# omerbt/TokenFlow

Measured on AMD Instinct MI355X. Metric: denoising-step hot-path frames/sec, higher is better.
Workload: dtype bf16

## Files before the change

### include/tokenflow_hip.h

```cpp
#ifndef TOKENFLOW_HIP_H
#define TOKENFLOW_HIP_H

#include <stddef.h>
#include <stdint.h>

#ifdef __cplusplus
extern "C" {
#endif

#define TF_ABI_VERSION 11

#define TF_API __attribute__((visibility("default")))

#define TF_BF16 0
#define TF_F16 1
#define TF_F32 2

#define TF_ATTN_INJECT 1
#define TF_ATTN_EXACT_SCALE 2
#define TF_ATTN_BANK_ONLY 4
#define TF_ATTN_SOURCE_ONLY 8
#define TF_ATTN_NO_SPLIT 16
#define TF_ATTN_FOLD_SCALE 64
#define TF_ATTN_OUT_F32 32
// ... 84 lines not shown
TF_API int tf_ext_attn_runs_merge_edits(void* out, int K, int Kq, int S, int H, int Dh, int n_runs, int n_edits,
                                 unsigned inject_mask, int64_t out_branch_stride, int64_t out_frame_stride,
                                 int flags, int dtype, void* ws, size_t ws_bytes, void* stream);

TF_API int tf_ext_attn_run_edits_plan(int K, int Kq, int run_n, int n_runs, int S, int H, int Dh, int n_edits,
                               unsigned inject_mask, int flags, int dtype, char* buf, size_t len);

TF_API int tf_head_pack(const void* const* slabs, const int64_t* frame_strides, int ns, void* send, int W, int Kl, int S,
                 int hd, int64_t ld, int elem_bytes, void* stream);

TF_API int tf_head_unpack(const void* recv, void* const* dsts, const int64_t* frame_strides, int nb, int W, int Kl, int S,
                   int hd, int64_t ld, int elem_bytes, void* stream);

TF_API int tf_window_halo_pack(const void* const* slabs, const int64_t* frame_strides, int ns, void* send, int n_seg,
                        const int* seg_f0, const int* seg_n, int Kl, int S, int D, int64_t ld, int dtype, void* stream);

TF_API int tf_frame_set_halo_pack(const void* const* slabs, const int64_t* frame_strides, int ns, void* send, int n_peer,
                           const uint64_t* masks, int Kl, int S, int D, int64_t ld, int dtype, void* stream);

TF_API int tf_edit_halo_pack(const void* const* slabs, const int64_t* frame_strides, int ns, void* send, int n_peer,
                      const uint64_t* masks, const void* const* q_slabs, const int64_t* q_frame_strides, int nq, void* q_stage,
                      int Kl, int S, int D, int64_t ld, int64_t ld_q, int dtype, void* stream);

TF_API int tf_pivot_inv_norm(const void* piv, float* inv_norm, int64_t rows, int D, int dtype,
                      void* stream);

TF_API size_t tf_nn_search_workspace_bytes(int64_t n_tgt, int S, int D, int P);

TF_API int tf_nn_search(const void* tgt, const void* piv, const float* inv_norm, int32_t* idx,
                 int64_t n_tgt, int S, int D, int P, int kf0, int kf1, int dtype,
                 void* ws, size_t ws_bytes, void* stream);

TF_API int tf_nn_search_plan(int64_t n_tgt, int S, int D, int P, int C, char* buf, size_t len);

TF_API int tf_gather_blend(const void* kf_out, const int32_t* idx, const float* w, const void* resid,
                    void* out, int K, int n, int S, int D, int P, int kf0, int kf1,
                    int in_dtype, int res_dtype, int out_dtype, void* stream);

TF_API size_t tf_nn_gather_blend_workspace_bytes(int64_t n_tgt, int S, int D, int P);

TF_API int tf_nn_gather_blend(const void* tgt, const void* piv, const float* inv_norm,
                       const void* kf_out, const float* w, const void* resid, void* out,
                       int K, int n, int S, int D, int P, int kf0, int kf1,
                       int search_dtype, int in_dtype, int res_dtype, int out_dtype,
                       void* ws, size_t ws_bytes, void* stream);

TF_API size_t tf_nn_gather_blend_chunks_workspace_bytes(int64_t n_tgt_chunk, int S, int D, int C);

TF_API int tf_nn_gather_blend_chunks(const void* tgt, const void* piv, const float* inv_norm, const void* kf_out,
                              const float* w, const void* resid, void* out, int K, int n, int C, int S, int D,
                              int slot0, int first_single, int search_dtype, int in_dtype, int res_dtype,
                              int out_dtype, int single_dtype, void* ws, size_t ws_bytes, void* stream);

TF_API int tf_nn_gather_blend_norm(const void* tgt, const void* piv, const float* inv_norm, const void* kf_out,
                            const float* w, const void* resid, void* out, int K, int n, int S, int D, int P, int kf0,
                            int kf1, int search_dtype, int in_dtype, int res_dtype, int out_dtype, const void* gamma,
                            const void* beta, float eps, int w_dtype, void* norm_out, int norm_dtype, void* ws,
                            size_t ws_bytes, void* stream);

TF_API int tf_nn_gather_blend_chunks_norm(const void* tgt, const void* piv, const float* inv_norm, const void* kf_out,
                                   const float* w, const void* resid, void* out, int K, int n, int C, int S, int D,
                                   int slot0, int first_single, int search_dtype, int in_dtype, int res_dtype,
                                   int out_dtype, int single_dtype, const void* gamma, const void* beta, float eps,
                                   int w_dtype, void* norm_out, int norm_dtype, void* ws, size_t ws_bytes,
                                   void* stream);

// ... 210 lines not shown
```

### tokenflow_amd/_lib.py

```python
import ctypes
import os

_HERE = os.path.dirname(os.path.abspath(__file__))
LIB_PATH = os.environ.get("TOKENFLOW_HIP_LIB") or os.path.join(_HERE, "libtokenflow_hip.so")

TF_BF16, TF_F16, TF_F32 = 0, 1, 2
TF_ATTN_INJECT, TF_ATTN_EXACT_SCALE, TF_ATTN_BANK_ONLY, TF_ATTN_SOURCE_ONLY, TF_ATTN_NO_SPLIT = 1, 2, 4, 8, 16
TF_ATTN_OUT_F32 = 32
TF_ATTN_FOLD_SCALE = 64
TF_ATTN_NO_FUSED, TF_ATTN_FUSED = 128, 1 << 17
TF_ATTN_HINT_QB2, TF_ATTN_PRECISE_P, TF_ATTN_NO_PRECISE_P = 1 << 14, 1 << 15, 1 << 16
TF_ATTN_MULTI_V, TF_ATTN_NO_MULTI_V = 1 << 19, 1 << 20
TF_ATTN_MULTI_V64 = 1 << 21
TF_ATTN_RUN_MULTI_V = 1 << 22
TF_ATTN_HINT_MIX = 1 << 18


def attn_hint(qw: int = 0, kw: int = 0, qb: int = 1) -> int:
    code = {0: 0, 1: 1, 2: 2, 4: 3, 8: 4}
    return (code[qw] << 8) | (code[kw] << 11) | (TF_ATTN_HINT_QB2 if qb == 2 else 0)


ABI_VERSION = 11
TF_MAX_EDITS = 8
TF_MAX_SEGMENTS = 8
TF_MAX_WINDOW_FRAMES = 64
TF_RANK_HEADS, TF_RANK_BANK, TF_RANK_SLOTS, TF_RANK_NO_HALO, TF_RANK_INV_NORM = 0, 1, 64, 16, 32
TF_RANK_BANK_RUNS = 2
TF_RANK_BANK_EDIT_RUNS = 3
TF_ERR_COMM = -6

_c = ctypes
_SIGNATURES = {
    "tf_abi_version": (_c.c_int, []),
    "tf_last_error": (_c.c_char_p, []),
    "tf_ext_attn_workspace_bytes": (_c.c_size_t, [_c.c_int] * 5),
    "tf_ext_attn_plan": (_c.c_int, [_c.c_int] * 7 + [_c.c_char_p, _c.c_size_t]),
    "tf_nn_search_plan": (_c.c_int, [_c.c_int64] + [_c.c_int] * 4 + [_c.c_char_p, _c.c_size_t]),
    "tf_ext_attn_fwd": (_c.c_int, [_c.c_void_p] * 4 + [_c.c_int] * 6 + [_c.c_int64, _c.c_float, _c.c_int, _c.c_int,
                                   _c.c_void_p, _c.c_size_t, _c.c_void_p]),
    "tf_ext_attn_fwd_strided": (_c.c_int, [_c.c_void_p] * 4 + [_c.c_int] * 6 + [_c.c_int64, _c.c_void_p, _c.c_float,
                                           _c.c_int, _c.c_int, _c.c_void_p, _c.c_size_t, _c.c_void_p]),
    "tf_ext_attn_edits_workspace_bytes": (_c.c_size_t, [_c.c_int] * 6),
    "tf_ext_attn_fwd_edits": (_c.c_int, [_c.c_void_p] * 4 + [_c.c_int] * 6 + [_c.c_int64, _c.c_void_p, _c.c_float,
                                         _c.c_int, _c.c_int, _c.c_int, _c.c_void_p, _c.c_size_t, _c.c_void_p]),
    "tf_ext_attn_edits_plan": (_c.c_int, [_c.c_int] * 8 + [_c.c_char_p, _c.c_size_t]),
    "tf_nn_gather_blend_chunks_edits": (_c.c_int, [_c.c_void_p] * 7 + [_c.c_int] * 13 + [_c.c_void_p, _c.c_size_t,
                                                   _c.c_void_p]),
    "tf_nn_gather_blend_chunks_norm_edits": (_c.c_int, [_c.c_void_p] * 7 + [_c.c_int] * 13 + [_c.c_void_p, _c.c_void_p,
                                                        _c.c_float, _c.c_int, _c.c_void_p, _c.c_int, _c.c_void_p,
                                                        _c.c_size_t, _c.c_void_p]),
    "tf_nn_gather_blend_edits_plan": (_c.c_int, [_c.c_int] * 6 + [_c.c_char_p, _c.c_size_t]),
    "tf_inject_copy_edits": (_c.c_int, [_c.c_void_p, _c.c_int64, _c.c_int, _c.c_int, _c.c_void_p]),
    "tf_ext_attn_fwd_edits_masked": (_c.c_int, [_c.c_void_p] * 4 + [_c.c_int] * 6 + [_c.c_int64, _c.c_void_p, _c.c_float,
                                                _c.c_int, _c.c_int, _c.c_int, _c.c_uint, _c.c_void_p, _c.c_size_t,
                                                _c.c_void_p]),
    "tf_ext_attn_edits_masked_plan": (_c.c_int, [_c.c_int] * 6 + [_c.c_uint, _c.c_int, _c.c_int, _c.c_char_p, _c.c_size_t]),
    "tf_ext_attn_fwd_edits_part": (_c.c_int, [_c.c_void_p] * 4 + [_c.c_int] * 6 + [_c.c_int64, _c.c_void_p, _c.c_float,
                                              _c.c_int, _c.c_int, _c.c_int, _c.c_uint, _c.c_int, _c.c_void_p, _c.c_size_t,
                                              _c.c_void_p]),
    "tf_ext_attn_edits_part_plan": (_c.c_int, [_c.c_int] * 6 + [_c.c_uint, _c.c_int, _c.c_int, _c.c_int, _c.c_char_p,
                                               _c.c_size_t]),
    "tf_inject_copy_edits_masked": (_c.c_int, [_c.c_void_p, _c.c_int64, _c.c_int, _c.c_uint, _c.c_int, _c.c_void_p]),
    "tf_ext_attn_runs_workspace_bytes": (_c.c_size_t, [_c.c_int] * 7),
    "tf_ext_attn_run": (_c.c_int, [_c.c_void_p] * 4 + [_c.c_int] * 10 + [_c.c_int64, _c.c_void_p, _c.c_float, _c.c_int,
                                   _c.c_int, _c.c_void_p, _c.c_size_t, _c.c_void_p]),
    "tf_ext_attn_runs_merge": (_c.c_int, [_c.c_void_p] + [_c.c_int] * 6 + [_c.c_int64, _c.c_int64, _c.c_int, _c.c_int,
                                          _c.c_void_p, _c.c_size_t, _c.c_void_p]),
    "tf_ext_attn_run_plan": (_c.c_int, [_c.c_int] * 9 + [_c.c_char_p, _c.c_size_t]),
    "tf_ext_attn_runs_edits_workspace_bytes": (_c.c_size_t, [_c.c_int] * 8),
    "tf_ext_attn_run_edits": (_c.c_int, [_c.c_void_p] * 4 + [_c.c_int] * 10 + [_c.c_int64, _c.c_void_p, _c.c_float, _c.c_int,
# ... 155 lines not shown
```

### tokenflow_amd/csrc/nn_search.hip

```cpp
#include <stdlib.h>

#include <type_traits>

#include "tf_common.h"

namespace {

template <int BK>
__device__ __forceinline__ int swz_off(int row, int piece) {
    if constexpr (BK == 64) return row * 128 + ((piece ^ ((row >> 1) & 7)) << 4);
    return row * (BK * 2) + ((piece ^ (row & 15)) << 4);
}

template <typename T>
__global__ __launch_bounds__(256) void pivot_inv_norm_kernel(const typename T::elem* __restrict__ piv,
                                                             float* __restrict__ inv_norm, int64_t rows, int D) {
    const int lane = threadIdx.x & 63;
    const int64_t wave = (int64_t)blockIdx.x * 4 + (threadIdx.x >> 6);
    const int64_t nwaves = (int64_t)gridDim.x * 4;
    for (int64_t r = wave; r < rows; r += nwaves) {
        const float inv = tf_row_inv_norm<T>(piv + r * D, D, lane);
        if (lane == 0) inv_norm[r] = inv;
    }
}

template <typename T, int WN, int BK, int TM>
__global__ __launch_bounds__(256) void nn_search_kernel(const typename T::elem* __restrict__ tgt,
                                                        const typename T::elem* __restrict__ piv,
                                                        const float* __restrict__ inv_norm,
                                                        int32_t* __restrict__ idx_out,
                                                        NnPartial* __restrict__ part_out, int64_t n_tgt, int S,
                                                        int D, int kf0, int kf1, int tiles_per_split, NnChunks ch) {
    typedef typename T::vec8 vec8;
    constexpr int TN = 64 * WN;
// ... 669 lines not shown
#pragma unroll
            for (int tt = 0; tt < TT; ++tt) {
                const float sc = acc[tt][r] * w;
                if (sc > best_v[tt]) {
                    best_v[tt] = sc;
                    best_i[tt] = (mt0 + mt) * TMR + rl;
                }
            }
        }
        if (has_next) stage_write(mt + 1);
        asm volatile("s_waitcnt vmcnt(0)" ::: "memory");
        __syncthreads();
    }
#pragma unroll
    for (int tt = 0; tt < TT; ++tt) {
        const float ov = __shfl_xor(best_v[tt], 32);
        const int oi = __shfl_xor(best_i[tt], 32);
        float bv = best_v[tt];
        int bi = best_i[tt];
        if (ov > bv || (ov == bv && oi < bi)) {
            bv = ov;
            bi = oi;
        }
        bi = bi < S ? bi : S - 1;
        if (hi == 0 && t_row[tt] < t_end) {
            if (part_out)
                part_out[((int64_t)blockIdx.z * gridDim.y + p) * n_tgt + t_row[tt]] = NnPartial{bv, bi};
            else
                idx_out[(int64_t)p * n_tgt + t_row[tt]] = bi;
        }
    }
}

template <typename T, int DK, int TJ = 4>
__global__ __launch_bounds__(256, TJ == 4 ? 2 : 3) void nn_search_rbs_kernel(const typename T::elem* __restrict__ tgt,
                                                               const typename T::elem* __restrict__ piv,
                                                               const float* __restrict__ inv_norm,
                                                               int32_t* __restrict__ idx_out,
                                                               NnPartial* __restrict__ part_out, int64_t n_tgt, int S,
                                                               int kf0, int kf1, int tiles_per_split, NnChunks ch) {
    typedef typename T::elem E;
    typedef typename T::vec8 vec8;
    constexpr int D = 16 * DK;
    constexpr int KS32 = D / 32;
    static_assert(D % 32 == 0 && (D / 8) % 8 == 0, "32-wide k-steps; the swizzle permutes inside groups of 8 pieces");
    constexpr int TMR = 32;
    constexpr int NPIECE = TMR * D * 2 / 1024;
    static_assert(NPIECE % 4 == 0, "pieces split evenly over the 4 waves");
    constexpr int A_ELEMS = TMR * D;

    extern __shared__ __attribute__((aligned(16))) unsigned char smem[];
    float* sInv = reinterpret_cast<float*>(smem + 2 * A_ELEMS * sizeof(E));

    const int tid = threadIdx.x;
    const int lane = tid & 63;
    const int wave = tid >> 6;
    const int g = lane >> 4;
    const int n16 = lane & 15;
    const int p = blockIdx.y;
    const int chunk = blockIdx.x / ch.ppc;
    if (p == 1 && nn_chunk_single(ch, chunk)) return;
    const int kf = (p == 0 ? kf0 : kf1) + chunk;
    const E* pv = piv + (int64_t)kf * S * D;
    const float* inv = inv_norm + (int64_t)kf * S;
    const int64_t t_end = (chunk + 1) * (int64_t)ch.nS;
    int64_t t_row[TJ];
#pragma unroll
    for (int j = 0; j < TJ; ++j)
        t_row[j] = chunk * (int64_t)ch.nS + (int64_t)(blockIdx.x - chunk * ch.ppc) * (64 * TJ) + wave * (16 * TJ) + 16 * j + n16;

    const int n_mt_all = (S + TMR - 1) / TMR;
    const int mt0 = blockIdx.z * tiles_per_split;
    const int n_mt = min(tiles_per_split, n_mt_all - mt0);

    vec8 fb[TJ][KS32];
#pragma unroll
    for (int j = 0; j < TJ; ++j) {
        const E* tp = tgt + (t_row[j] < t_end ? t_row[j] : t_end - 1) * D + 8 * g;
#pragma unroll
        for (int t = 0; t < KS32; ++t) fb[j][t] = __builtin_bit_cast(vec8, ld16(tp + 32 * t));
    }

    typedef __attribute__((address_space(3))) void* lds_ptr;
    typedef const __attribute__((address_space(1))) void* glb_ptr;
    const int wave_u = __builtin_amdgcn_readfirstlane(wave);
    int a_off[NPIECE / 4];
#pragma unroll
    for (int i = 0; i < NPIECE / 4; ++i) {
        const int o = (wave_u + 4 * i) * 1024 + lane * 16;
        const int r = o / (2 * D), pos = (o - r * 2 * D) >> 4;
        a_off[i] = r * D + ((pos ^ ((r >> 1) & 7)) << 3);
    }
    float rinv = 0.f;
    const unsigned lds0 = (unsigned)(size_t)(lds_ptr)smem;
    auto stage_load = [&](int mt) {
        const E* tile = pv + (int64_t)(mt0 + mt) * TMR * D;
#pragma unroll
        for (int i = 0; i < NPIECE / 4; ++i) {
            const unsigned dst = __builtin_amdgcn_readfirstlane(lds0 + (mt & 1) * (A_ELEMS * (int)sizeof(E)) + (wave_u + 4 * i) * 1024);
            unsigned keep;
            asm volatile("s_mov_b32 %0, m0\n\ts_mov_b32 m0, %2\n\ts_nop 0\n\tglobal_load_lds_dwordx4 %1, off\n\ts_mov_b32 m0, %0"
                         : "=&s"(keep)
                         : "v"((glb_ptr)(tile + a_off[i])), "s"(dst)
                         : "memory");
        }
        if (tid < TMR) {
            int row = (mt0 + mt) * TMR + tid;
            rinv = inv[row < S ? row : S - 1];
        }
    };
    auto stage_write = [&](int mt) {
        if (tid < TMR) sInv[(mt & 1) * TMR + tid] = rinv;
    };
    auto tile_done = [&]() {
        asm volatile("" : "+v"(rinv));
        asm volatile("s_waitcnt vmcnt(0)" ::: "memory");
        __syncthreads();
    };

    constexpr int ROW_BYTES = D * (int)sizeof(E);
    constexpr int HALF_BYTES = 16 * ROW_BYTES;
    constexpr int A_BYTES = A_ELEMS * (int)sizeof(E);
    constexpr int RING = TJ == 4 ? 3 : 5;
    static_assert(TMR == 32 && sizeof(E) == 2, "two 16-row halves whose rows 16 i + n16 share (r >> 1) & 7; 8 elements per 16-B piece");
    static_assert(KS32 % 2 == 0, "k-steps pair up into groups of 8 pieces");
    static_assert((KS32 / 2 - 1) * 128 + HALF_BYTES + A_BYTES < 65536, "every fragment offset fits ds_read's 16-bit immediate");
    static_assert(RING - 1 <= KS32, "the ring's prologue stays inside phase A");
    const int fa_base[2] = {n16 * ROW_BYTES + ((g ^ ((n16 >> 1) & 7)) << 4), n16 * ROW_BYTES + (((4 + g) ^ ((n16 >> 1) & 7)) << 4)};
    auto frag = [&](const int (&cur)[2], int k) {
        const int t = k % KS32, i = k / KS32;
        return __builtin_bit_cast(vec8, ld16(smem + cur[t & 1] + (t >> 1) * 128 + i * HALF_BYTES));
    };

    float best_v[TJ];
    int best_i[TJ];
#pragma unroll
    for (int j = 0; j < TJ; ++j) best_v[j] = -INFINITY, best_i[j] = 0;
    stage_load(0);
    stage_write(0);
#pragma unroll
    for (int j = 0; j < TJ; ++j)
#pragma unroll
        for (int t = 0; t < KS32; ++t) asm volatile("" : "+v"(fb[j][t]));
    asm volatile("" ::"s"(idx_out), "s"(part_out));
    tile_done();
    constexpr int EPG = TJ / 2;
    static_assert(TJ % 2 == 0 && EPG * (KS32 - 2) >= 4 * TJ, "a half-tile's fold fits beside the inner groups of a phase");
    auto fold1 = [&](const f32x4 (&a)[TJ], const f32x4 w, const int row0, int e) {
        const int r = e / TJ, j = e % TJ;
        asm volatile("" : "+v"(best_v[j]), "+v"(best_i[j]));
        const float sc = a[j][r] * w[r];
        if (sc > best_v[j]) {
            best_v[j] = sc;
            best_i[j] = row0 + r;
        }
        asm volatile("" : "+v"(best_v[j]), "+v"(best_i[j]));
    };
    f32x4 acc0[TJ], acc1[TJ];
#pragma unroll
    for (int j = 0; j < TJ; ++j) acc1[j] = f32x4{-INFINITY, -INFINITY, -INFINITY, -INFINITY};
    f32x4 w0, w1 = f32x4{1.f, 1.f, 1.f, 1.f};
    int row0, row1 = 0;
    vec8 fa[RING];
    int cur[2];
    auto group = [&](int k, f32x4 (&acc)[TJ], const f32x4 (&accf)[TJ], const f32x4 wf, const int rowf) {
        const int t = k % KS32;
        const bool read = k + RING - 1 < 2 * KS32;
        if (read) fa[(k + RING - 1) % RING] = frag(cur, k + RING - 1);
#pragma unroll
        for (int j = 0; j < TJ; ++j)
            acc[j] = T::mfma16(fa[k % RING], fb[j][t], t == 0 ? f32x4{0.f, 0.f, 0.f, 0.f} : acc[j]);
        if (t >= 1 && t <= (4 * TJ) / EPG) {
#pragma unroll
            for (int e = (t - 1) * EPG; e < t * EPG; ++e) fold1(accf, wf, rowf, e);
        }
        if (read) __builtin_amdgcn_sched_group_barrier(0x100, 1, 0);
#pragma unroll
        for (int j = 0; j < TJ; ++j) {
            __builtin_amdgcn_sched_group_barrier(0x008, 1, 0);
            __builtin_amdgcn_sched_group_barrier(0x002, 2, 0);
        }
        __builtin_amdgcn_sched_barrier(0);
    };
    for (int mt = 0; mt < n_mt; ++mt) {
        const bool has_next = mt + 1 < n_mt;
        const int buf = (mt & 1) * A_BYTES;
        cur[0] = fa_base[0] + buf, cur[1] = fa_base[1] + buf;
        const float* si = sInv + (mt & 1) * TMR + 4 * g;
#pragma unroll
        for (int k = 0; k < RING - 1; ++k) fa[k] = frag(cur, k);
        w0 = *reinterpret_cast<const f32x4*>(si);
        if (has_next) stage_load(mt + 1);
        row0 = (mt0 + mt) * TMR + 4 * g;
        __builtin_amdgcn_sched_barrier(0);
#pragma unroll
        for (int k = 0; k < KS32; ++k) group(k, acc0, acc1, w1, row1);
        w1 = *reinterpret_cast<const f32x4*>(si + 16);
#pragma unroll
        for (int k = KS32; k < 2 * KS32; ++k) group(k, acc1, acc0, w0, row0);
        row1 = row0 + 16;
        if (has_next) stage_write(mt + 1);
        tile_done();
    }
#pragma unroll
    for (int e = 0; e < 4 * TJ; ++e) fold1(acc1, w1, row1, e);
#pragma unroll
    for (int j = 0; j < TJ; ++j) {
        float bv = best_v[j];
        int bi = best_i[j];
#pragma unroll
        for (int o_ = 16; o_ <= 32; o_ <<= 1) {
            const float ov = __shfl_xor(bv, o_);
            const int oi = __shfl_xor(bi, o_);
            if (ov > bv || (ov == bv && oi < bi)) {
                bv = ov;
                bi = oi;
            }
        }
        bi = bi < S ? bi : S - 1;
        if (g == 0 && t_row[j] < t_end) {
            if (part_out)
                part_out[((int64_t)blockIdx.z * gridDim.y + p) * n_tgt + t_row[j]] = NnPartial{bv, bi};
            else
                idx_out[(int64_t)p * n_tgt + t_row[j]] = bi;
        }
    }
}

__global__ __launch_bounds__(256) void nn_finalize_kernel(const NnPartial* __restrict__ part,
                                                          int32_t* __restrict__ idx_out, int64_t total, int splits) {
    const int64_t g = (int64_t)blockIdx.x * 256 + threadIdx.x;
    if (g >= total) return;
    NnPartial b = part[g];
    for (int s = 1; s < splits; ++s) {
        const NnPartial c = part[(int64_t)s * total + g];
        if (c.v > b.v || (c.v == b.v && c.i < b.i)) b = c;
    }
    idx_out[g] = b.i;
}

enum NnKernel {
    NN_RB,
    NN_RB2,
    NN_WIDE,
    NN_BK64,
    NN_BK128,
    NN_DEEP,
    NN_GLDS
};
struct NnPlan {
    int kern;
    int64_t panels;
    int splits, tiles_per_split;
};

static int nn_min_wgs(int C) {
    static const int env = [] {
// ... 86 lines not shown
    auto kern = nn_search_kernel<T, WN, BK, TM>;
    (void)hipFuncSetAttribute(reinterpret_cast<const void*>(kern), hipFuncAttributeMaxDynamicSharedMemorySize, (int)lds);
    const NnChunks ch = nn_chunks(n_tgt, (int)pl.panels, single_mask);
    hipLaunchKernelGGL(kern, grid, dim3(256), lds, st, reinterpret_cast<const typename T::elem*>(tgt),
                       reinterpret_cast<const typename T::elem*>(piv), inv_norm, idx,
                       (splits > 1 || !fin) ? ws : nullptr, n_tgt * C, S, D, kf0, kf1, tps, ch);
    TF_LAUNCH_CHECK("tf_nn_search");
    return (fin && splits > 1) ? finalize(ws, idx, n_tgt * C * P, splits, st) : 0;
}

template <typename T>
int launch_nn_glds(const void* tgt, const void* piv, const float* inv_norm, int32_t* idx, NnPartial* ws, int64_t n_tgt,
                   int S, int D, int P, int kf0, int kf1, hipStream_t st, bool fin, int C, uint64_t single_mask) {
    constexpr size_t lds = 2 * (256 + 256) * 64 * 2 + 2 * 256 * 4 + 4 * 256 * 8;
    static_assert(lds <= 160 * 1024, "LDS");
    const NnPlan pl = nn_plan(n_tgt, S, D, P, C);
    const int splits = pl.splits, tps = pl.tiles_per_split;
    dim3 grid((unsigned)(pl.panels * C), (unsigned)P, (unsigned)splits);
    if (tf_plan_note("glds[splits=%d%s]", splits, C > 1 ? ",chunks" : "")) return (fin && splits > 1) ? finalize(ws, idx, n_tgt * C * P, splits, st) : 0;
#ifndef TF_TUNE_NN_NO_GLDS_SH
    auto kern = nn_search_glds_kernel<T, true>;
#else
    auto kern = nn_search_glds_kernel<T, false>;
#endif
    (void)hipFuncSetAttribute(reinterpret_cast<const void*>(kern), hipFuncAttributeMaxDynamicSharedMemorySize, (int)lds);
    const NnChunks ch = nn_chunks(n_tgt, (int)pl.panels, single_mask);
    hipLaunchKernelGGL(kern, grid, dim3(512), lds, st, reinterpret_cast<const typename T::elem*>(tgt),
                       reinterpret_cast<const typename T::elem*>(piv), inv_norm, idx,
                       (splits > 1 || !fin) ? ws : nullptr, n_tgt * C, S, D, kf0, kf1, tps, ch);
    TF_LAUNCH_CHECK("tf_nn_search");
    return (fin && splits > 1) ? finalize(ws, idx, n_tgt * C * P, splits, st) : 0;
}

template <typename T, int DK>
int launch_nn_rb(const void* tgt, const void* piv, const float* inv_norm, int32_t* idx, NnPartial* ws, int64_t n_tgt,
                 int S, int P, int kf0, int kf1, hipStream_t st, bool fin, int C, uint64_t single_mask) {
    constexpr int D = 16 * DK;
    const size_t lds = 2 * 32 * (D + 8) * 2 + 2 * 32 * 4;
    const NnPlan pl = nn_plan(n_tgt, S, D, P, C);
    const int splits = pl.splits, tps = pl.tiles_per_split;
    dim3 grid((unsigned)(pl.panels * C), (unsigned)P, (unsigned)splits);
    const NnChunks ch = nn_chunks(n_tgt, (int)pl.panels, single_mask);
    if (pl.kern == NN_RB2) {
        const size_t lds_g = 2 * 32 * D * 2 + 2 * 32 * 4;
#ifndef TF_TUNE_NN_NO_RBS
        if (tf_plan_note("rbs<TJ=4>[splits=%d%s]", splits, C > 1 ? ",chunks" : "")) return (fin && splits > 1) ? finalize(ws, idx, n_tgt * C * P, splits, st) : 0;
        hipLaunchKernelGGL((nn_search_rbs_kernel<T, DK>), grid, dim3(256), lds_g, st,
                           reinterpret_cast<const typename T::elem*>(tgt), reinterpret_cast<const typename T::elem*>(piv),
                           inv_norm, idx, (splits > 1 || !fin) ? ws : nullptr, n_tgt * C, S, kf0, kf1, tps, ch);
        TF_LAUNCH_CHECK("tf_nn_search");
        return (fin && splits > 1) ? finalize(ws, idx, n_tgt * C * P, splits, st) : 0;
#endif
        if (tf_plan_note("rbg<TT=2>[splits=%d%s]", splits, C > 1 ? ",chunks" : "")) return (fin && splits > 1) ? finalize(ws, idx, n_tgt * C * P, splits, st) : 0;
        hipLaunchKernelGGL((nn_search_rbg_kernel<T, DK, 2>), grid, dim3(256), lds_g, st,
                           reinterpret_cast<const typename T::elem*>(tgt), reinterpret_cast<const typename T::elem*>(piv),
                           inv_norm, idx, (splits > 1 || !fin) ? ws : nullptr, n_tgt * C, S, kf0, kf1, tps, ch);
        TF_LAUNCH_CHECK("tf_nn_search");
        return (fin && splits > 1) ? finalize(ws, idx, n_tgt * C * P, splits, st) : 0;
    }
    static const bool dma = [] { const char* e = getenv("TF_NN_RB_GLDS"); return !e || atoi(e) != 0; }();
    if (dma && S % 32 == 0) {
        const size_t lds_g = 2 * 32 * D * 2 + 2 * 32 * 4;
#ifndef TF_TUNE_NN_NO_RBS
        if (tf_plan_note("rbs<TJ=2>[splits=%d%s]", splits, C > 1 ? ",chunks" : "")) return (fin && splits > 1) ? finalize(ws, idx, n_tgt * C * P, splits, st) : 0;
        hipLaunchKernelGGL((nn_search_rbs_kernel<T, DK, 2>), grid, dim3(256), lds_g, st,
                           reinterpret_cast<const typename T::elem*>(tgt), reinterpret_cast<const typename T::elem*>(piv),
                           inv_norm, idx, (splits > 1 || !fin) ? ws : nullptr, n_tgt * C, S, kf0, kf1, tps, ch);
        TF_LAUNCH_CHECK("tf_nn_search");
        return (fin && splits > 1) ? finalize(ws, idx, n_tgt * C * P, splits, st) : 0;
#endif
        if (tf_plan_note("rbg<TT=1>[splits=%d%s]", splits, C > 1 ? ",chunks" : "")) return (fin && splits > 1) ? finalize(ws, idx, n_tgt * C * P, splits, st) : 0;
        hipLaunchKernelGGL((nn_search_rbg_kernel<T, DK>), grid, dim3(256), lds_g, st,
                           reinterpret_cast<const typename T::elem*>(tgt), reinterpret_cast<const typename T::elem*>(piv),
                           inv_norm, idx, (splits > 1 || !fin) ? ws : nullptr, n_tgt * C, S, kf0, kf1, tps, ch);
        TF_LAUNCH_CHECK("tf_nn_search");
        return (fin && splits > 1) ? finalize(ws, idx, n_tgt * C * P, splits, st) : 0;
    }
    if (tf_plan_note("rb[splits=%d%s]", splits, C > 1 ? ",chunks" : "")) return (fin && splits > 1) ? finalize(ws, idx, n_tgt * C * P, splits, st) : 0;
    hipLaunchKernelGGL((nn_search_rb_kernel<T, DK>), grid, dim3(256), lds, st,
                       reinterpret_cast<const typename T::elem*>(tgt), reinterpret_cast<const typename T::elem*>(piv),
                       inv_norm, idx, (splits > 1 || !fin) ? ws : nullptr, n_tgt * C, S, kf0, kf1, tps, ch);
    TF_LAUNCH_CHECK("tf_nn_search");
    return (fin && splits > 1) ? finalize(ws, idx, n_tgt * C * P, splits, st) : 0;
}

template <typename T>
int dispatch_nn(const void* tgt, const void* piv, const float* inv_norm, int32_t* idx, NnPartial* ws, int64_t n_tgt,
                int S, int D, int P, int kf0, int kf1, hipStream_t st, bool fin, int C = 1, uint64_t single_mask = 0) {
    TF_ARG(n_tgt <= (int64_t)INT32_MAX, TF_ERR_SHAPE, "tf_nn_search: %lld targets per chunk (< 2^31)", (long long)n_tgt);
    switch (nn_plan(n_tgt, S, D, P, C).kern) {
        case NN_RB:
        case NN_RB2:
            return launch_nn_rb<T, 20>(tgt, piv, inv_norm, idx, ws, n_tgt, S, P, kf0, kf1, st, fin, C, single_mask);
        case NN_GLDS:
            return launch_nn_glds<T>(tgt, piv, inv_norm, idx, ws, n_tgt, S, D, P, kf0, kf1, st, fin, C, single_mask);
        case NN_WIDE:
            return launch_nn<T, 2, 64, 128>(tgt, piv, inv_norm, idx, ws, n_tgt, S, D, P, kf0, kf1, st, fin, C, single_mask);
        case NN_DEEP:
            return launch_nn<T, 1, 256, 64>(tgt, piv, inv_norm, idx, ws, n_tgt, S, D, P, kf0, kf1, st, fin, C, single_mask);
        case NN_BK128:
// ... 6 lines not shown
}

extern "C" int tf_pivot_inv_norm(const void* piv, float* inv_norm, int64_t rows, int D, int dtype, void* stream) {
    TF_ARG(piv && inv_norm, TF_ERR_NULL, "tf_pivot_inv_norm: null pointer");
    TF_ARG(dtype == TF_BF16 || dtype == TF_F16, TF_ERR_DTYPE, "tf_pivot_inv_norm: dtype %d (bf16/f16 only)", dtype);
    TF_ARG(rows > 0 && D > 0 && D % 8 == 0, TF_ERR_SHAPE, "tf_pivot_inv_norm: rows=%lld D=%d (D %% 8 == 0)",
           (long long)rows, D);
    TF_ARG(tf_aligned16(piv), TF_ERR_ALIGN, "tf_pivot_inv_norm: piv not 16-byte aligned");
    hipStream_t st = reinterpret_cast<hipStream_t>(stream);
    const unsigned grid = (unsigned)((rows + 3) / 4 < 4096 ? (rows + 3) / 4 : 4096);
    if (dtype == TF_BF16)
        hipLaunchKernelGGL(pivot_inv_norm_kernel<BF16>, dim3(grid), dim3(256), 0, st,
                           reinterpret_cast<const __bf16*>(piv), inv_norm, rows, D);
    else
        hipLaunchKernelGGL(pivot_inv_norm_kernel<F16>, dim3(grid), dim3(256), 0, st,
                           reinterpret_cast<const _Float16*>(piv), inv_norm, rows, D);
    TF_LAUNCH_CHECK("tf_pivot_inv_norm");
    return 0;
}

extern "C" int tf_nn_search_plan(int64_t n_tgt, int S, int D, int P, int C, char* buf, size_t len) {
    TF_ARG(n_tgt > 0 && S > 0 && D > 0 && D % 8 == 0 && (P == 1 || P == 2) && C >= 1 && (C == 1 || P == 2), TF_ERR_SHAPE,
           "tf_nn_search_plan: n_tgt=%lld S=%d D=%d P=%d C=%d", (long long)n_tgt, S, D, P, C);
    TfPlanRec rec{buf, len, 0, 0};
    if (buf && len) buf[0] = 0;
    tf_plan_rec = &rec;
    const int rc = dispatch_nn<BF16>(nullptr, nullptr, nullptr, nullptr, nullptr, n_tgt, S, D, P, 0, 1, nullptr, C == 1, C, 0);
    tf_plan_rec = nullptr;
    if (rc) return rc;
    TF_ARG(rec.used < len, TF_ERR_WORKSPACE, "tf_nn_search_plan: the plan needs %zu bytes", rec.used + 1);
    return rec.n;
}

extern "C" size_t tf_nn_search_workspace_bytes(int64_t n_tgt, int S, int D, int P) {
    if (n_tgt <= 0 || S <= 0 || D <= 0 || P <= 0) return 0;
    const NnPlan pl = nn_plan(n_tgt, S, D, P);
    const size_t bytes = pl.splits > 1 ? (size_t)pl.splits * P * n_tgt * sizeof(NnPartial) : 0;
    return bytes < 256 ? 256 : bytes;
}

extern "C" int tf_nn_search(const void* tgt, const void* piv, const float* inv_norm, int32_t* idx, int64_t n_tgt,
                            int S, int D, int P, int kf0, int kf1, int dtype, void* ws, size_t ws_bytes,
                            void* stream) {
    TF_ARG(tgt && piv && inv_norm && idx && ws, TF_ERR_NULL, "tf_nn_search: null pointer");
    TF_ARG(dtype == TF_BF16 || dtype == TF_F16, TF_ERR_DTYPE, "tf_nn_search: dtype %d (bf16/f16 only)", dtype);
    TF_ARG(n_tgt > 0 && S > 0 && D > 0 && D % 8 == 0 && (P == 1 || P == 2) && kf0 >= 0 && (P == 1 || kf1 >= 0),
           TF_ERR_SHAPE, "tf_nn_search: n_tgt=%lld S=%d D=%d P=%d kf=(%d,%d)", (long long)n_tgt, S, D, P, kf0, kf1);
    TF_ARG(tf_aligned16(tgt) && tf_aligned16(piv) && tf_aligned16(ws) && tf_aligned16(inv_norm), TF_ERR_ALIGN,
           "tf_nn_search: inputs not 16-byte aligned (inv_norm included: the LDS-DMA kernel fetches it in 16-byte pieces)");
    TF_ARG(ws_bytes >= tf_nn_search_workspace_bytes(n_tgt, S, D, P), TF_ERR_WORKSPACE,
           "tf_nn_search: workspace %zu < %zu bytes", ws_bytes, tf_nn_search_workspace_bytes(n_tgt, S, D, P));
    hipStream_t st = reinterpret_cast<hipStream_t>(stream);
    NnPartial* part = reinterpret_cast<NnPartial*>(ws);
    return dtype == TF_BF16 ? dispatch_nn<BF16>(tgt, piv, inv_norm, idx, part, n_tgt, S, D, P, kf0, kf1, st, true)
                            : dispatch_nn<F16>(tgt, piv, inv_norm, idx, part, n_tgt, S, D, P, kf0, kf1, st, true);
}

int tf_nn_search_partials(const void* tgt, const void* piv, const float* inv_norm, NnPartial* part, int64_t n_tgt,
                          int S, int D, int P, int kf0, int kf1, int dtype, hipStream_t st, int* splits, int C,
                          uint64_t single_mask) {
    *splits = nn_plan(n_tgt, S, D, P, C).splits;
    return dtype == TF_BF16
               ? dispatch_nn<BF16>(tgt, piv, inv_norm, nullptr, part, n_tgt, S, D, P, kf0, kf1, st, false, C, single_mask)
               : dispatch_nn<F16>(tgt, piv, inv_norm, nullptr, part, n_tgt, S, D, P, kf0, kf1, st, false, C, single_mask);
}

// ... 4 lines not shown
```

### tokenflow_amd/ops.py

```python
import ctypes
import os
from typing import Optional, Sequence

import torch

from . import _lib

_DT = {torch.bfloat16: _lib.TF_BF16, torch.float16: _lib.TF_F16, torch.float32: _lib.TF_F32}


def _need_gpu(*ts):
    dev = None
    for t in ts:
        if t is None:
            continue
        if not t.is_cuda:
            raise _lib.TokenflowHipError(
                "tokenflow_amd ops run on MI355X only: got a CPU tensor (there is no CPU fallback)")
        if dev is None:
            dev = t.device
        elif t.device != dev:
            raise _lib.TokenflowHipError(f"tokenflow_amd ops: tensors on different devices ({dev} and {t.device})")
    return dev

# ... 256 lines not shown
    if part not in ("bank", "all"):
        raise ValueError(f"attn_frame_sets_part_plan: part {part!r} (\"bank\" or \"all\": the source part is set-free)")
    tab = _frame_sets("attn_frame_sets_part_plan", sets, K, Kq, int(q_frame0))
    flags = _attn_flags(inject, part, out_dtype == torch.float32, False, no_split, fused, hints)
    return _plan_tokens("tf_ext_attn_frame_sets_part_plan", _lib.load().tf_ext_attn_frame_sets_part_plan, K, Kq, int(q_frame0), S,
                        heads, dh, flags, _DT[dtype], ctypes.cast(tab, ctypes.c_void_p))


def attn_frame_sets_edits_plan(K: int, sets, S: int, heads: int, dh: int, n_edits: int, inject_mask: int,
                               dtype: torch.dtype = torch.bfloat16, out_dtype: Optional[torch.dtype] = None,
                               no_split: Optional[bool] = None, fused: Optional[bool] = None, multi_v: Optional[bool] = None,
                               multi_v64: Optional[bool] = None, hints: int = 0) -> list:
    tab = _frame_sets("attn_frame_sets_edits_plan", sets, K, K)
    mask = _edit_mask("attn_frame_sets_edits_plan", inject_mask, n_edits)
    flags = _attn_flags(False, "all", out_dtype == torch.float32, False, no_split, fused, hints) | _multi_v_bits(multi_v, multi_v64)
    return _plan_tokens("tf_ext_attn_frame_sets_edits_plan", _lib.load().tf_ext_attn_frame_sets_edits_plan, K, K, 0, S, heads,
                        dh, int(n_edits), mask, flags, _DT[dtype], ctypes.cast(tab, ctypes.c_void_p))


def _single_mask(what: str, mask, C: int) -> int:
    m = int(mask)
    if not 1 <= C <= 64 or m < 0 or m >> C:
        raise ValueError(f"{what}: single_mask {m:#x} over {C} chunks (1 .. 64 chunks, no bit at or above them)")
    return m


def propagate_segments_plan(n: int, n_chunks: int, S: int, D: int, single_mask: int) -> list:
    return _plan_tokens("tf_nn_gather_blend_segments_plan", _lib.load().tf_nn_gather_blend_segments_plan, int(n),
                        int(n_chunks), S, D, _single_mask("propagate_segments_plan", single_mask, int(n_chunks)))


def nn_plan(n_tgt: int, S: int, D: int, P: int, C: int = 1) -> list:
    return _plan_tokens("tf_nn_search_plan", _lib.load().tf_nn_search_plan, int(n_tgt), S, D, P, C)


def ext_attn(q: torch.Tensor, k: torch.Tensor, v: torch.Tensor, heads: int, scale: float,
             inject: bool, out: Optional[torch.Tensor] = None, q_frame0: int = 0,
             fold_scale: Optional[bool] = None, part: str = "all",
             out_dtype: Optional[torch.dtype] = None, no_split: Optional[bool] = None,
             fused: Optional[bool] = None, hints: int = 0) -> torch.Tensor:
    dev = _need_gpu(q, k, v, out)
    lib = _lib.load()
    B, S, D = k.shape
    Bq = q.shape[0]
    if B % 3 or Bq % 3 or D % heads or q.shape[1:] != k.shape[1:] or v.shape != k.shape:
        raise ValueError(f"ext_attn: bad shapes q{tuple(q.shape)} k{tuple(k.shape)} v{tuple(v.shape)} heads {heads}")
    K, Kq, dh = B // 3, Bq // 3, D // heads
    dt = _DT.get(q.dtype)
    if dt is None or dt == _lib.TF_F32 or k.dtype != q.dtype or v.dtype != q.dtype:
        raise TypeError(f"ext_attn: q/k/v must share dtype bf16 or f16, got {q.dtype},{k.dtype},{v.dtype}")

    def rows(t):
        if t.stride(-1) != 1 or t.stride(0) != S * t.stride(1):
            t = t.contiguous()
        return t
    q, k, v = rows(q), rows(k), rows(v)
    ld = q.stride(1)
    if k.stride(1) != ld or v.stride(1) != ld:
        q, k, v = q.contiguous(), k.contiguous(), v.contiguous()
        ld = D
    if out_dtype is None:
        out_dtype = out.dtype if out is not None else q.dtype
    if out_dtype not in (q.dtype, torch.float32):
        raise TypeError(f"ext_attn: out_dtype {out_dtype} (the input dtype or float32)")
    if out is None:
        out = torch.empty(Bq, S, D, dtype=out_dtype, device=q.device)
# ... 1214 lines not shown
```

Measured before the change: 1654.

## Balance nearest-neighbour search work across resident workgroups with flattened tile runs

Adds a balanced mode for the row-block nearest-neighbour search kernel. The (chunk, pivot, panel, tile) space is flattened into equal-length runs sized to the number of resident workgroups, so each workgroup walks consecutive tiles across pivot-frame and panel boundaries. At each boundary it emits a partial result and reloads target rows only when they change. Block indices are remapped across the eight XCDs. The aim is to cut tail imbalance and partially filled waves when the split grid does not match CU occupancy, at the cost of more complex control flow, duplicated partial writes for split slots, and a device-attribute query.

```diff
diff --git a/include/tokenflow_hip.h b/include/tokenflow_hip.h
--- a/include/tokenflow_hip.h
+++ b/include/tokenflow_hip.h
@@ -140,6 +140,8 @@
                  void* ws, size_t ws_bytes, void* stream);
 
 TF_API int tf_nn_search_plan(int64_t n_tgt, int S, int D, int P, int C, char* buf, size_t len);
+
+TF_API int tf_nn_search_partition(int64_t n_tgt, int S, int D, int P, int C, uint64_t single_mask, int cus, int* out);
 
 TF_API int tf_gather_blend(const void* kf_out, const int32_t* idx, const float* w, const void* resid,
                     void* out, int K, int n, int S, int D, int P, int kf0, int kf1,
diff --git a/tokenflow_amd/_lib.py b/tokenflow_amd/_lib.py
--- a/tokenflow_amd/_lib.py
+++ b/tokenflow_amd/_lib.py
@@ -37,6 +37,7 @@
     "tf_ext_attn_workspace_bytes": (_c.c_size_t, [_c.c_int] * 5),
     "tf_ext_attn_plan": (_c.c_int, [_c.c_int] * 7 + [_c.c_char_p, _c.c_size_t]),
     "tf_nn_search_plan": (_c.c_int, [_c.c_int64] + [_c.c_int] * 4 + [_c.c_char_p, _c.c_size_t]),
+    "tf_nn_search_partition": (_c.c_int, [_c.c_int64] + [_c.c_int] * 4 + [_c.c_uint64, _c.c_int, _c.POINTER(_c.c_int)]),
     "tf_ext_attn_fwd": (_c.c_int, [_c.c_void_p] * 4 + [_c.c_int] * 6 + [_c.c_int64, _c.c_float, _c.c_int, _c.c_int,
                                    _c.c_void_p, _c.c_size_t, _c.c_void_p]),
     "tf_ext_attn_fwd_strided": (_c.c_int, [_c.c_void_p] * 4 + [_c.c_int] * 6 + [_c.c_int64, _c.c_void_p, _c.c_float,
diff --git a/tokenflow_amd/csrc/nn_search.hip b/tokenflow_amd/csrc/nn_search.hip
--- a/tokenflow_amd/csrc/nn_search.hip
+++ b/tokenflow_amd/csrc/nn_search.hip
@@ -1,5 +1,6 @@
 #include <stdlib.h>
 
+#include <algorithm>
 #include <type_traits>
 
 #include "tf_common.h"
@@ -735,13 +736,20 @@
     }
 }
 
-template <typename T, int DK, int TJ = 4>
+constexpr int NN_XCDS = 8;
+struct NnRuns {
+    int total;
+    int P;
+    int slots;
+};
+template <typename T, int DK, int TJ = 4, bool BAL = false>
 __global__ __launch_bounds__(256, TJ == 4 ? 2 : 3) void nn_search_rbs_kernel(const typename T::elem* __restrict__ tgt,
                                                                const typename T::elem* __restrict__ piv,
                                                                const float* __restrict__ inv_norm,
                                                                int32_t* __restrict__ idx_out,
                                                                NnPartial* __restrict__ part_out, int64_t n_tgt, int S,
-                                                               int kf0, int kf1, int tiles_per_split, NnChunks ch) {
+                                                               int kf0, int kf1, int tiles_per_split, NnChunks ch,
+                                                               NnRuns runs) {
     typedef typename T::elem E;
     typedef typename T::vec8 vec8;
     constexpr int D = 16 * DK;
@@ -760,29 +768,59 @@
     const int wave = tid >> 6;
     const int g = lane >> 4;
     const int n16 = lane & 15;
-    const int p = blockIdx.y;
-    const int chunk = blockIdx.x / ch.ppc;
-    if (p == 1 && nn_chunk_single(ch, chunk)) return;
-    const int kf = (p == 0 ? kf0 : kf1) + chunk;
-    const E* pv = piv + (int64_t)kf * S * D;
-    const float* inv = inv_norm + (int64_t)kf * S;
-    const int64_t t_end = (chunk + 1) * (int64_t)ch.nS;
-    int64_t t_row[TJ];
-#pragma unroll
-    for (int j = 0; j < TJ; ++j)
-        t_row[j] = chunk * (int64_t)ch.nS + (int64_t)(blockIdx.x - chunk * ch.ppc) * (64 * TJ) + wave * (16 * TJ) + 16 * j + n16;
-
     const int n_mt_all = (S + TMR - 1) / TMR;
-    const int mt0 = blockIdx.z * tiles_per_split;
-    const int n_mt = min(tiles_per_split, n_mt_all - mt0);
+    int p, chunk, panel, mt0, n_mt, slot;
+    if constexpr (!BAL) {
+        p = blockIdx.y;
+        chunk = blockIdx.x / ch.ppc;
+        panel = blockIdx.x - chunk * ch.ppc;
+        if (p == 1 && nn_chunk_single(ch, chunk)) return;
+        mt0 = blockIdx.z * tiles_per_split;
+        n_mt = min(tiles_per_split, n_mt_all - mt0);
+        slot = blockIdx.z;
+    } else {
+        const int run = (blockIdx.x % NN_XCDS) * (gridDim.x / NN_XCDS) + blockIdx.x / NN_XCDS;
+        const int start = run * tiles_per_split;
+        if (start >= runs.total) return;
+        n_mt = min(tiles_per_split, runs.total - start);
+        int q = start / n_mt_all;
+        mt0 = start - q * n_mt_all;
+        slot = 0;
+        for (int t = mt0; t > 0; t -= tiles_per_split) ++slot;
+        chunk = 0;
+        for (;;) {
+            const int np = (runs.P == 2 && !nn_chunk_single(ch, chunk)) ? 2 * ch.ppc : ch.ppc;
+            if (q < np) break;
+            q -= np;
+            if ((int64_t)(++chunk) * ch.nS >= n_tgt) return;
+        }
+        const bool two = runs.P == 2 && !nn_chunk_single(ch, chunk);
+        panel = two ? q >> 1 : q;
+        p = two ? q & 1 : 0;
+    }
+    const E* pv;
+    const float* inv;
+    {
+        const int kf = (p == 0 ? kf0 : kf1) + chunk;
+        pv = piv + (int64_t)kf * S * D;
+        inv = inv_norm + (int64_t)kf * S;
+    }
+    auto target_row = [&](int c, int pn, int j) {
+        return c * (int64_t)ch.nS + (int64_t)pn * (64 * TJ) + wave * (16 * TJ) + 16 * j + n16;
+    };
 
     vec8 fb[TJ][KS32];
-#pragma unroll
-    for (int j = 0; j < TJ; ++j) {
-        const E* tp = tgt + (t_row[j] < t_end ? t_row[j] : t_end - 1) * D + 8 * g;
-#pragma unroll
-        for (int t = 0; t < KS32; ++t) fb[j][t] = __builtin_bit_cast(vec8, ld16(tp + 32 * t));
-    }
+    auto load_targets = [&](int c, int pn) {
+        const int64_t t_end = (c + 1) * (int64_t)ch.nS;
+#pragma unroll
+        for (int j = 0; j < TJ; ++j) {
+            const int64_t t_row = target_row(c, pn, j);
+            const E* tp = tgt + (t_row < t_end ? t_row : t_end - 1) * D + 8 * g;
+#pragma unroll
+            for (int t = 0; t < KS32; ++t) fb[j][t] = __builtin_bit_cast(vec8, ld16(tp + 32 * t));
+        }
+    };
+    load_targets(chunk, panel);
 
     typedef __attribute__((address_space(3))) void* lds_ptr;
     typedef const __attribute__((address_space(1))) void* glb_ptr;
@@ -796,8 +834,8 @@
     }
     float rinv = 0.f;
     const unsigned lds0 = (unsigned)(size_t)(lds_ptr)smem;
-    auto stage_load = [&](int mt) {
-        const E* tile = pv + (int64_t)(mt0 + mt) * TMR * D;
+    auto stage_load = [&](const E* pvx, const float* invx, int tl, int mt) {
+        const E* tile = pvx + (int64_t)tl * TMR * D;
 #pragma unroll
         for (int i = 0; i < NPIECE / 4; ++i) {
             const unsigned dst = __builtin_amdgcn_readfirstlane(lds0 + (mt & 1) * (A_ELEMS * (int)sizeof(E)) + (wave_u + 4 * i) * 1024);
@@ -808,8 +846,8 @@
                          : "memory");
         }
         if (tid < TMR) {
-            int row = (mt0 + mt) * TMR + tid;
-            rinv = inv[row < S ? row : S - 1];
+            int row = tl * TMR + tid;
+            rinv = invx[row < S ? row : S - 1];
         }
     };
     auto stage_write = [&](int mt) {
@@ -839,13 +877,17 @@
     int best_i[TJ];
 #pragma unroll
     for (int j = 0; j < TJ; ++j) best_v[j] = -INFINITY, best_i[j] = 0;
-    stage_load(0);
+    stage_load(pv, inv, mt0, 0);
     stage_write(0);
-#pragma unroll
-    for (int j = 0; j < TJ; ++j)
-#pragma unroll
-        for (int t = 0; t < KS32; ++t) asm volatile("" : "+v"(fb[j][t]));
+    auto targets_settled = [&]() {
+#pragma unroll
+        for (int j = 0; j < TJ; ++j)
+#pragma unroll
+            for (int t = 0; t < KS32; ++t) asm volatile("" : "+v"(fb[j][t]));
+    };
+    targets_settled();
     asm volatile("" ::"s"(idx_out), "s"(part_out));
+    if constexpr (BAL) asm volatile("" ::"s"(runs.slots), "s"(runs.P), "s"(kf0), "s"(kf1), "s"(tgt));
     tile_done();
     constexpr int EPG = TJ / 2;
     static_assert(TJ % 2 == 0 && EPG * (KS32 - 2) >= 4 * TJ, "a half-tile's fold fits beside the inner groups of a phase");
@@ -885,16 +927,44 @@
         }
         __builtin_amdgcn_sched_barrier(0);
     };
-    for (int mt = 0; mt < n_mt; ++mt) {
-        const bool has_next = mt + 1 < n_mt;
+    auto finish = [&](int pp, int c, int pn, int s0, int s1) {
+#pragma unroll
+        for (int e = 0; e < 4 * TJ; ++e) fold1(acc1, w1, row1, e);
+        const int64_t t_end = (c + 1) * (int64_t)ch.nS;
+        const int P = BAL ? runs.P : (int)gridDim.y;
+#pragma unroll
+        for (int j = 0; j < TJ; ++j) {
+            float bv = best_v[j];
+            int bi = best_i[j];
+#pragma unroll
+            for (int o_ = 16; o_ <= 32; o_ <<= 1) {
+                const float ov = __shfl_xor(bv, o_);
+                const int oi = __shfl_xor(bi, o_);
+                if (ov > bv || (ov == bv && oi < bi)) {
+                    bv = ov;
+                    bi = oi;
+                }
+            }
+            bi = bi < S ? bi : S - 1;
+            const int64_t t_row = target_row(c, pn, j);
+            if (g == 0 && t_row < t_end) {
+                if (part_out) {
+                    for (int s = s0; s < s1; ++s) part_out[((int64_t)s * P + pp) * n_tgt + t_row] = NnPartial{bv, bi};
+                } else {
+                    idx_out[(int64_t)pp * n_tgt + t_row] = bi;
+                }
+            }
+        }
+    };
+    auto tile_step = [&](int mt, int tl, bool has_next, const E* pvx, const float* invx, int tl_n) {
         const int buf = (mt & 1) * A_BYTES;
         cur[0] = fa_base[0] + buf, cur[1] = fa_base[1] + buf;
         const float* si = sInv + (mt & 1) * TMR + 4 * g;
 #pragma unroll
         for (int k = 0; k < RING - 1; ++k) fa[k] = frag(cur, k);
         w0 = *reinterpret_cast<const f32x4*>(si);
-        if (has_next) stage_load(mt + 1);
-        row0 = (mt0 + mt) * TMR + 4 * g;
+        if (has_next) stage_load(pvx, invx, tl_n, mt + 1);
+        row0 = tl * TMR + 4 * g;
         __builtin_amdgcn_sched_barrier(0);
 #pragma unroll
         for (int k = 0; k < KS32; ++k) group(k, acc0, acc1, w1, row1);
@@ -904,28 +974,43 @@
         row1 = row0 + 16;
         if (has_next) stage_write(mt + 1);
         tile_done();
-    }
-#pragma unroll
-    for (int e = 0; e < 4 * TJ; ++e) fold1(acc1, w1, row1, e);
-#pragma unroll
-    for (int j = 0; j < TJ; ++j) {
-        float bv = best_v[j];
-        int bi = best_i[j];
-#pragma unroll
-        for (int o_ = 16; o_ <= 32; o_ <<= 1) {
-            const float ov = __shfl_xor(bv, o_);
-            const int oi = __shfl_xor(bi, o_);
-            if (ov > bv || (ov == bv && oi < bi)) {
-                bv = ov;
-                bi = oi;
-            }
-        }
-        bi = bi < S ? bi : S - 1;
-        if (g == 0 && t_row[j] < t_end) {
-            if (part_out)
-                part_out[((int64_t)blockIdx.z * gridDim.y + p) * n_tgt + t_row[j]] = NnPartial{bv, bi};
-            else
-                idx_out[(int64_t)p * n_tgt + t_row[j]] = bi;
+    };
+    if constexpr (!BAL) {
+        for (int mt = 0; mt < n_mt; ++mt) tile_step(mt, mt0 + mt, mt + 1 < n_mt, pv, inv, mt0 + mt + 1);
+        finish(p, chunk, panel, slot, slot + 1);
+    } else {
+        int left = n_mt, mt = 0, tile = mt0;
+        for (;;) {
+            bool same_targets;
+            do {
+                const int seg_n = min(left, n_mt_all - tile);
+                const bool pair_end = tile + seg_n == n_mt_all;
+                int p_n = 0, chunk_n = chunk, panel_n = panel;
+                if (runs.P == 2 && p == 0 && !nn_chunk_single(ch, chunk)) {
+                    p_n = 1;
+                } else if (++panel_n == ch.ppc) {
+                    panel_n = 0, ++chunk_n;
+                }
+                const int kf_n = (p_n == 0 ? kf0 : kf1) + chunk_n;
+                const E* pv_n = piv + (int64_t)kf_n * S * D;
+                const float* inv_n = inv_norm + (int64_t)kf_n * S;
+                for (int i = 0; i + 1 < seg_n; ++i, ++tile, ++mt) tile_step(mt, tile, true, pv, inv, tile + 1);
+                tile_step(mt, tile, left > seg_n, pv_n, inv_n, 0);
+                ++mt;
+                finish(p, chunk, panel, slot, pair_end ? runs.slots : slot + 1);
+                left -= seg_n;
+#pragma unroll
+                for (int j = 0; j < TJ; ++j) {
+                    best_v[j] = -INFINITY, best_i[j] = 0;
+                    acc1[j] = f32x4{-INFINITY, -INFINITY, -INFINITY, -INFINITY};
+                }
+                same_targets = panel_n == panel && chunk_n == chunk;
+                p = p_n, chunk = chunk_n, panel = panel_n, pv = pv_n, inv = inv_n;
+                tile = 0, slot = 0;
+            } while (left > 0 && same_targets);
+            if (left <= 0) break;
+            load_targets(chunk, panel);
+            targets_settled();
         }
     }
 }
@@ -1078,6 +1163,65 @@
     return (fin && splits > 1) ? finalize(ws, idx, n_tgt * C * P, splits, st) : 0;
 }
 
+struct NnPartition {
+    int balanced;
+    int G, R;
+    int total;
+};
+
+static int nn_rbs_form(const NnPlan& pl, int S) {
+#ifdef TF_TUNE_NN_NO_RBS
+    return 0;
+#endif
+    if (pl.kern == NN_RB2) return 4;
+    static const bool dma = [] { const char* e = getenv("TF_NN_RB_GLDS"); return !e || atoi(e) != 0; }();
+    return (pl.kern == NN_RB && dma && S % 32 == 0) ? 2 : 0;
+}
+
+static int nn_device_cus() {
+    static int cache[64];
+    int dev = 0;
+    if (hipGetDevice(&dev) != hipSuccess) {
+        (void)hipGetLastError();
+        return 0;
+    }
+    int cus = (dev >= 0 && dev < 64) ? __atomic_load_n(&cache[dev], __ATOMIC_RELAXED) : 0;
+    if (cus <= 0) {
+        if (hipDeviceGetAttribute(&cus, hipDeviceAttributeMultiprocessorCount, dev) != hipSuccess) {
+            (void)hipGetLastError();
+            return 0;
+        }
+        if (dev >= 0 && dev < 64) __atomic_store_n(&cache[dev], cus, __ATOMIC_RELAXED);
+    }
+    return cus;
+}
+
+static NnPartition nn_partition(const NnPlan& pl, int tj, int64_t n_tgt, int S, int P, int C, uint64_t single_mask, int cus) {
+    NnPartition pt{0, 0, 0, 0};
+    static const int mode = [] { const char* e = getenv("TF_SEARCH_BALANCED"); return e ? atoi(e) : 1; }();
+    if (mode == 0 || tj == 0 || cus <= 0 || S % 32 != 0) return pt;
+    if (mode == 1 && (pl.splits == 1 || (tj == 2 && pl.tiles_per_split >= 24))) return pt;
+    const int n_tiles = S / 32;
+    int64_t pairs = 0;
+    for (int c = 0; c < C; ++c) pairs += pl.panels * ((P == 2 && !(c < 64 && ((single_mask >> c) & 1))) ? 2 : 1);
+    const int64_t total = pairs * n_tiles;
+    if (pairs <= 0 || total >= (int64_t)INT32_MAX) return pt;
+    const int64_t resident = (int64_t)(tj == 4 ? 2 : 3) * cus;
+    const int64_t grid_wgs = std::max<int64_t>(1, total / pl.tiles_per_split);
+    const int64_t g0 = std::min(resident, grid_wgs);
+    int64_t R;
+    if (pl.splits == 1) {
+        R = ((pairs + g0 - 1) / g0) * n_tiles;
+    } else {
+        R = std::max<int64_t>((total + g0 - 1) / g0, (n_tiles + pl.splits - 2) / (pl.splits - 1));
+    }
+    pt.balanced = 1;
+    pt.R = (int)R;
+    pt.G = (int)((total + R - 1) / R);
+    pt.total = (int)total;
+    return pt;
+}
+
 template <typename T, int DK>
 int launch_nn_rb(const void* tgt, const void* piv, const float* inv_norm, int32_t* idx, NnPartial* ws, int64_t n_tgt,
                  int S, int P, int kf0, int kf1, hipStream_t st, bool fin, int C, uint64_t single_mask) {
@@ -1091,9 +1235,17 @@
         const size_t lds_g = 2 * 32 * D * 2 + 2 * 32 * 4;
 #ifndef TF_TUNE_NN_NO_RBS
         if (tf_plan_note("rbs<TJ=4>[splits=%d%s]", splits, C > 1 ? ",chunks" : "")) return (fin && splits > 1) ? finalize(ws, idx, n_tgt * C * P, splits, st) : 0;
-        hipLaunchKernelGGL((nn_search_rbs_kernel<T, DK>), grid, dim3(256), lds_g, st,
-                           reinterpret_cast<const typename T::elem*>(tgt), reinterpret_cast<const typename T::elem*>(piv),
-                           inv_norm, idx, (splits > 1 || !fin) ? ws : nullptr, n_tgt * C, S, kf0, kf1, tps, ch);
+        const NnPartition pt = nn_partition(pl, 4, n_tgt, S, P, C, single_mask, nn_device_cus());
+        if (pt.balanced)
+            hipLaunchKernelGGL((nn_search_rbs_kernel<T, DK, 4, true>), dim3((unsigned)((pt.G + NN_XCDS - 1) / NN_XCDS * NN_XCDS)), dim3(256), lds_g, st,
+                               reinterpret_cast<const typename T::elem*>(tgt), reinterpret_cast<const typename T::elem*>(piv),
+                               inv_norm, idx, (splits > 1 || !fin) ? ws : nullptr, n_tgt * C, S, kf0, kf1, pt.R, ch,
+                               NnRuns{pt.total, P, splits});
+        else
+            hipLaunchKernelGGL((nn_search_rbs_kernel<T, DK>), grid, dim3(256), lds_g, st,
+                               reinterpret_cast<const typename T::elem*>(tgt), reinterpret_cast<const typename T::elem*>(piv),
+                               inv_norm, idx, (splits > 1 || !fin) ? ws : nullptr, n_tgt * C, S, kf0, kf1, tps, ch,
+                               NnRuns{0, P, splits});
         TF_LAUNCH_CHECK("tf_nn_search");
         return (fin && splits > 1) ? finalize(ws, idx, n_tgt * C * P, splits, st) : 0;
 #endif
@@ -1109,9 +1261,17 @@
         const size_t lds_g = 2 * 32 * D * 2 + 2 * 32 * 4;
 #ifndef TF_TUNE_NN_NO_RBS
         if (tf_plan_note("rbs<TJ=2>[splits=%d%s]", splits, C > 1 ? ",chunks" : "")) return (fin && splits > 1) ? finalize(ws, idx, n_tgt * C * P, splits, st) : 0;
-        hipLaunchKernelGGL((nn_search_rbs_kernel<T, DK, 2>), grid, dim3(256), lds_g, st,
-                           reinterpret_cast<const typename T::elem*>(tgt), reinterpret_cast<const typename T::elem*>(piv),
-                           inv_norm, idx, (splits > 1 || !fin) ? ws : nullptr, n_tgt * C, S, kf0, kf1, tps, ch);
+        const NnPartition pt = nn_partition(pl, 2, n_tgt, S, P, C, single_mask, nn_device_cus());
+        if (pt.balanced)
+            hipLaunchKernelGGL((nn_search_rbs_kernel<T, DK, 2, true>), dim3((unsigned)((pt.G + NN_XCDS - 1) / NN_XCDS * NN_XCDS)), dim3(256), lds_g, st,
+                               reinterpret_cast<const typename T::elem*>(tgt), reinterpret_cast<const typename T::elem*>(piv),
+                               inv_norm, idx, (splits > 1 || !fin) ? ws : nullptr, n_tgt * C, S, kf0, kf1, pt.R, ch,
+                               NnRuns{pt.total, P, splits});
+        else
+            hipLaunchKernelGGL((nn_search_rbs_kernel<T, DK, 2>), grid, dim3(256), lds_g, st,
+                               reinterpret_cast<const typename T::elem*>(tgt), reinterpret_cast<const typename T::elem*>(piv),
+                               inv_norm, idx, (splits > 1 || !fin) ? ws : nullptr, n_tgt * C, S, kf0, kf1, tps, ch,
+                               NnRuns{0, P, splits});
         TF_LAUNCH_CHECK("tf_nn_search");
         return (fin && splits > 1) ? finalize(ws, idx, n_tgt * C * P, splits, st) : 0;
 #endif
@@ -1184,6 +1344,21 @@
     return rec.n;
 }
 
+extern "C" int tf_nn_search_partition(int64_t n_tgt, int S, int D, int P, int C, uint64_t single_mask, int cus, int* out) {
+    TF_ARG(out, TF_ERR_NULL, "tf_nn_search_partition: null pointer");
+    TF_ARG(n_tgt > 0 && n_tgt <= (int64_t)INT32_MAX && S > 0 && D > 0 && D % 8 == 0 && (P == 1 || P == 2) && C >= 1 &&
+               (C == 1 || P == 2),
+           TF_ERR_SHAPE, "tf_nn_search_partition: n_tgt=%lld S=%d D=%d P=%d C=%d", (long long)n_tgt, S, D, P, C);
+    const NnPlan pl = nn_plan(n_tgt, S, D, P, C);
+    const int tj = nn_rbs_form(pl, S);
+    const NnPartition pt = nn_partition(pl, tj, n_tgt, S, P, C, single_mask, (cus > 0 || tj == 0) ? cus : nn_device_cus());
+    out[0] = pt.balanced;
+    out[1] = pt.balanced ? pt.G : (int)std::min<int64_t>(pl.panels * C * P * pl.splits, INT32_MAX);
+    out[2] = pt.balanced ? pt.R : pl.tiles_per_split;
+    out[3] = pl.splits;
+    return 0;
+}
+
 extern "C" size_t tf_nn_search_workspace_bytes(int64_t n_tgt, int S, int D, int P) {
     if (n_tgt <= 0 || S <= 0 || D <= 0 || P <= 0) return 0;
     const NnPlan pl = nn_plan(n_tgt, S, D, P);
diff --git a/tokenflow_amd/ops.py b/tokenflow_amd/ops.py
--- a/tokenflow_amd/ops.py
+++ b/tokenflow_amd/ops.py
@@ -312,6 +312,13 @@
 
 def nn_plan(n_tgt: int, S: int, D: int, P: int, C: int = 1) -> list:
     return _plan_tokens("tf_nn_search_plan", _lib.load().tf_nn_search_plan, int(n_tgt), S, D, P, C)
+
+
+def nn_partition(n_tgt: int, S: int, D: int, P: int, C: int = 1, single_mask: int = 0, cus: int = 0) -> dict:
+    out = (ctypes.c_int * 4)()
+    _lib.check(_lib.load().tf_nn_search_partition(int(n_tgt), S, D, P, C, int(single_mask), int(cus), out),
+               "tf_nn_search_partition")
+    return {"balanced": bool(out[0]), "G": out[1], "R": out[2], "splits": out[3]}
 
 
 def ext_attn(q: torch.Tensor, k: torch.Tensor, v: torch.Tensor, heads: int, scale: float,
```

Result: no change. 1659, median of 6 (+0.3%).
